# diaoenmao/Multimodal-Controller-for-Generative-Models

Hardware: AMD Instinct MI355X
Metric: images/sec (train step) MCGAN CIFAR-10 32x32 (higher is better)
Workload: dtype bf16

## Files before the change

### include/mcgen_hip.h

```cpp
#ifndef MCGEN_HIP_H
#define MCGEN_HIP_H

#include <stdint.h>

#ifdef __cplusplus
extern "C" {
#endif

enum { MCGEN_F32 = 0, MCGEN_BF16 = 1 };

const char* mcgen_last_error(void);
int mcgen_abi_version(void);

typedef struct {
    const void*  x;
    const float* scale;
    const float* shift;
    const float* code;
    const int16_t* cmap;
    int32_t C;
    int32_t ups;
    int32_t relu;
    int32_t ksize;
    int32_t group_n;
    int32_t cmap_stride;
    int32_t Cw;
    int32_t reserved_;
} mcgen_seg_t;

typedef struct {
    mcgen_seg_t  seg[2];
    int32_t      nseg;
    const void*  w;
    const float* bias;
    void*        y;
    int32_t N, H, W;
    int32_t Cout;
    int32_t Cout_w;
    int32_t Cy;
    int32_t pool;
    float   alpha;
    const void*  res;
    const float* ocode;
    const void*  gate_x;
    const float* gscale; const float* gshift; const float* gmean; const float* grstd;
    int32_t tanh_out;
    float*  stats;
    int32_t stats_mode;
    int32_t w_layout;
    const int16_t* ycmap;
    int32_t ycmap_stride;
    int32_t y_group;
    const float* bias2;
    const int32_t* wsel;
    int64_t wsel_stride;
    const int32_t* order;
    const int16_t* yperm;
    int32_t yperm_stride, reserved_;
} mcgen_conv_t;

enum { MCGEN_ROUTE_TILED = 0,
       MCGEN_ROUTE_MC, MCGEN_ROUTE_GK, MCGEN_ROUTE_GK_PP,
       MCGEN_ROUTE_SKINNY, MCGEN_ROUTE_SMAP, MCGEN_ROUTE_PX1, MCGEN_ROUTE_C8, MCGEN_ROUTE_HEAD };
typedef struct {
    int32_t route;
    int32_t form;
    int32_t bm, bn, pipe;
    int32_t m_tiles;
    int32_t grid_x, grid_y, threads, lds_bytes, a_bytes, grouped;
} mcgen_conv_plan_t;
int mcgen_conv_plan(const mcgen_conv_t* p, int dtype, mcgen_conv_plan_t* out);
int mcgen_conv_m_tiles(const mcgen_conv_t* p, int dtype);
int mcgen_conv_tile(const mcgen_conv_t* p, int dtype, int* bm, int* bn);
int mcgen_conv_form(const mcgen_conv_t* p, int dtype);
int mcgen_conv_fused(const mcgen_conv_t* p, int dtype, void* stream);

typedef struct {
    mcgen_seg_t  seg;
    const void*  dy;
    int32_t N, H, W;
    int32_t Cout, Cout_w, Cdy;
    int32_t dy_ups;
    float*  slabs;
    int32_t splits;
    int32_t halves;
    float*  bias_slabs;
} mcgen_wgrad_t;

int64_t mcgen_wgrad_slab_elems(const mcgen_wgrad_t* p);
int mcgen_wgrad(const mcgen_wgrad_t* p, int dtype, void* stream);
int mcgen_wgrad_c8_ok(const mcgen_wgrad_t* p, int dtype);
// ... 347 lines not shown
```

### multimodal-controller-for-generative-models_amd/csrc/conv_fused.hip

```cpp
#include "conv_tile.h"
#include <stdlib.h>
#include <type_traits>

namespace {

template <typename T, int BM, int BN, int WM, int WN>
struct ConvCfg {
    static constexpr int NT = 64 * WM * WN;
    static constexpr int FM = BM / WM / 16;
    static constexpr int FN = BN / WN / 16;
    static constexpr int ESZ = Elem<T>::BYTES;
    static constexpr int APITCH = MCGEN_CK * ESZ + 16 * ESZ;
    static constexpr int BROW = MCGEN_CK * ESZ;
    static constexpr int BBYTES = BN * BROW;
    static constexpr int EP = BN + 4;
    static constexpr int NI = (BM * 9 + NT - 1) / NT;
    static constexpr int UPR = BROW / 16;
    static constexpr int UNITS = BN * UPR;
    static constexpr int NU = (UNITS + NT - 1) / NT;
    static constexpr int EPX = (BN >= 128 && BM > 64) ? BM / 64 : 1;
    static constexpr int PPX = BM / EPX;
    static constexpr int CH = BN / 8;
    static constexpr int PROWS = NT / CH;
    static_assert(NT % CH == 0, "epilogue thread mapping");
// ... 1613 lines not shown
    int wset = 0;
    if (p.order || p.wsel) {
        const int tpi = (H * W) / BM, pos = tile_m / tpi;
        if (p.wsel) wset = p.wsel[pos];
        if (p.order) tile_m = p.order[pos] * tpi + (tile_m - pos * tpi);
    }
    const int cout0 = blockIdx.y * BN;
    const Geo g = make_geo(BM, tile_m, H, W);
    const int n_img = g.n0 < N ? g.n0 : N - 1;

    f32x4 acc[FN][FM];
#pragma unroll
    for (int i = 0; i < FN; ++i)
#pragma unroll
        for (int j = 0; j < FM; ++j) acc[i][j] = f32x4{0.f, 0.f, 0.f, 0.f};

    const mcgen_seg_t sg0 = seg_for_tile(p.seg[0], g);
    const int C0 = sg0.C;
    const char* wimg = reinterpret_cast<const char*>(p.w) + (size_t)wset * (size_t)p.wsel_stride * 2;
    const size_t wblock_bytes = (size_t)p.Cout_w * BROW;
    auto seg_info = [&](int si, const int16_t*& cidx, int& cw, int& cnt) {
        const mcgen_seg_t& sg = p.seg[si];
        cw = sg.Cw > 0 ? sg.Cw : sg.C;
        cidx = nullptr; cnt = sg.C;
        if (sg.cmap) {
            const int16_t* rec = sg.cmap + (size_t)n_img * sg.cmap_stride;
            cidx = rec + cw;
            cnt = (int)mc_sload(rec + 2 * cw + 32 + 2 * ((cw + 31) >> 5));
            if (cnt > sg.C) cnt = sg.C;
        }
    };
    const int16_t* cidx0 = nullptr; int cw0 = C0, cnt0 = C0;
    if constexpr (GK) seg_info(0, cidx0, cw0, cnt0);
    const int nchunk = GK ? ((cnt0 + 31) >> 5) : (C0 >> 5), T0 = nchunk * 9;
    const size_t tapstride0 = (size_t)(cw0 + 1) * p.Cout_w * 2;

    constexpr int UPR = C::UPR, RPP = 64 / UPR;
    int d_src[PPW];
    int k0_[PPW];
    const int rsub = lane / LPR, ci = lane % LPR;
#pragma unroll
    for (int k = 0; k < PPW; ++k) {
        const int piece = wave * PPW + k;
        if constexpr (!GK) {
            const int row = piece * RPP + lane / UPR, pu = lane % UPR;
            const int lgrp = pu ^ (3 * ((row >> 3) & 1));
            d_src[k] = (cout0 + row < p.Cout_w) ? (cout0 + row) * BROW + lgrp * 16 : (lane % UPR) * 16;
            k0_[k] = 0;
        } else {
            const int rho0 = RPPK * piece, rho = rho0 + rsub;
            k0_[k] = (rho0 < 16) ? 8 * (rho0 >> 2) + (rho0 & 3) : 8 * ((rho0 - 16) >> 2) + 4 + ((rho0 - 16) & 3);
            int co = cout0 + 16 * ((ci >> 1) ^ (rho & 7)) + 8 * (ci & 1);
            if (co > p.Cout_w - 8) co = p.Cout_w - 8;
            d_src[k] = co * 2;
        }
    }
    auto ksel_map = [&](const int16_t* cidx, int t, int k) -> int {
        const uint32_t d01 = mc_sload(cidx + 32 * t + k0_[k]);
        uint32_t sel = d01;
        if constexpr (RPPK == 4) {
            const uint32_t d23 = mc_sload(cidx + 32 * t + k0_[k] + 2);
            sel = (rsub & 2) ? d23 : d01;
        }
        return (int)((rsub & 1) ? (sel >> 16) : (sel & 0xffffu));
    };
    auto ksel = [&](const int16_t* cidx, int cw, int t, int k) -> int {
        if (cidx) return ksel_map(cidx, t, k);
// ... 164 lines not shown
                    for (int i = 0; i < HF; ++i) M::run(wf[fn], af[cs][i], acc[fn][i]);
            } else {
                const int sn = (slot_c + 1 == R) ? 0 : slot_c + 1;
                const char* ldsB = ldsB0 + sn * BB;
#pragma unroll
                for (int fn = 0; fn < FN; ++fn) {
#pragma unroll
                    for (int i = 0; i < HF; ++i) M::run(wf[fn], af[cs][i], acc[fn][HF + i]);
                    wf[fn] = wfrag(ldsB, fn);
                }
            }
            if constexpr (h == 0) {
                asm volatile("s_waitcnt lgkmcnt(0)" ::: "memory");
                pp_wait_vm<pp_vmcnt_b(ph, R, NIW, PPW)>();
                pp_barrier();
            } else {
                slot_c = (slot_c + 1 == R) ? 0 : slot_c + 1;
                ++tcur;
            }
        });
        if constexpr (GK) {
#pragma unroll
            for (int kk = 0; kk < PPW; ++kk) krow_c[kk] = krow_n[kk];
        }
    }
    asm volatile("s_waitcnt vmcnt(0)" ::: "memory");
    }

    if (p.nseg > 1) {
        int tg = 0;
        int nrest = 0;
        const int16_t* cidx1 = nullptr; int cw1 = 8, cnt1 = 0;
        if constexpr (GK) { seg_info(1, cidx1, cw1, cnt1); nrest = (cnt1 + 31) >> 5; }
        else for (int s = 1; s < p.nseg; ++s) nrest += (p.seg[s].C + MCGEN_CK - 1) / MCGEN_CK;
        const char* wseg1 = wimg + 9 * tapstride0;
        const size_t tapstride1 = (size_t)(cw1 + 1) * p.Cout_w * 2;
        auto tail_dma = [&](int t, int slot) {
#pragma unroll
            for (int k = 0; k < PPW; ++k) {
                if constexpr (GK) dma_piece_gk(wseg1, tapstride1, ksel(cidx1, cw1, t, k) * p.Cout_w * 2 + d_src[k], 0, slot, k);
                else dma_piece(T0 + t, slot, k);
            }
        };
        pp_barrier();
        constexpr int SUBW = BM * APITCH;
        constexpr int A2 = 2 * (((PP * APITCH + 1023) / 1024) * 1024);
        constexpr int TGMAX = (A2 + 2 * BB) / SUBW;
#ifndef MCGEN_PP_TG
#define MCGEN_PP_TG 4
#endif
        constexpr int TG = TGMAX < MCGEN_PP_TG ? TGMAX : MCGEN_PP_TG;
        constexpr int NI1 = (BM * 4 + NT - 1) / NT;
        static_assert(TG >= 1 && R >= 5, "tail groups: windows over the window buffers + two ring slots, weights in slots 2 .. 4");
        auto tslot = [](int t) { return 2 + t % 3; };
        auto tail_dma_c = [&](int t) { tail_dma(t < nrest ? t : nrest - 1, tslot(t)); };
        if (nrest > 0) { tail_dma_c(0); tail_dma_c(1); }
        for (int s = 1; s < p.nseg; ++s) {
            const mcgen_seg_t sg = seg_for_tile(p.seg[s], g);
            PatchStager<T, NT, NI1, APITCH> stager;
            stager.setup(sg, g, N, H, W, tid);
            const int b_lane = (wm * (BM / WM) + l15) * APITCH + lg * 16;
            const int nch = GK ? nrest : (sg.C + MCGEN_CK - 1) / MCGEN_CK;
#pragma unroll 1
            for (int q0 = 0; q0 < nch; q0 += TG) {
                const int ng = (nch - q0) < TG ? (nch - q0) : TG;
                if (q0 > 0) __builtin_amdgcn_s_barrier();
                {
                    typename PatchStager<T, NT, NI1, APITCH>::raw_t raw[TG];
#pragma unroll
                    for (int i = 0; i < TG; ++i) if (i < ng) stager.load(sg, (q0 + i) * MCGEN_CK, raw[i]);
#pragma unroll
                    for (int i = 0; i < TG; ++i) if (i < ng) stager.write(sg, (q0 + i) * MCGEN_CK, raw[i], ldsA0 + i * SUBW, g.n0 < N ? g.n0 : -1);
                }
#pragma unroll 1
                for (int i = 0; i < ng; ++i) {
                    if constexpr (PPW == 2) asm volatile("s_waitcnt vmcnt(2)" ::: "memory"); else asm volatile("s_waitcnt vmcnt(1)" ::: "memory");
                    asm volatile("s_waitcnt lgkmcnt(0)" ::: "memory");
                    pp_barrier();
                    tail_dma_c(tg + 2);
                    const char* ldsB = ldsB0 + tslot(tg) * BB;
                    const char* ldsW = ldsA0 + i * SUBW + b_lane;
                    typename M::frag xf[FM], yf[FN];
#pragma unroll
                    for (int fm = 0; fm < FM; ++fm) xf[fm] = *reinterpret_cast<const typename M::frag*>(ldsW + fm * 16 * APITCH);
#pragma unroll
                    for (int fn = 0; fn < FN; ++fn) yf[fn] = wfrag(ldsB, fn);
#pragma unroll
                    for (int fn = 0; fn < FN; ++fn)
#pragma unroll
                        for (int fm = 0; fm < FM; ++fm) M::run(yf[fn], xf[fm], acc[fn][fm]);
                    ++tg;
                }
            }
        }
    }
// ... 293 lines not shown
        r.route = MCGEN_ROUTE_C8;
    } else if (mcgen_conv_head_ok(p, dtype)) {
        r.route = MCGEN_ROUTE_HEAD;
    }
    const long Mtot = (long)p->N * p->H * p->W;
    r.m_tiles = r.route == MCGEN_ROUTE_SMAP ? p->N : bm > 0 ? (int)((Mtot + bm - 1) / bm) : 0;
    return r;
}
static int route_form(const Route& r) { return r.route >= MCGEN_ROUTE_SKINNY ? r.route - MCGEN_ROUTE_SKINNY + 1 : 0; }

static int validate(const mcgen_conv_t* p, bool launching) {
    MCGEN_CHECK(p && p->nseg >= 1 && p->nseg <= 2, "conv_fused: nseg must be 1 or 2");
    MCGEN_CHECK(p->N > 0 && ilog2_exact(p->H) >= 0 && ilog2_exact(p->W) >= 0, "conv_fused: H and W must be powers of two (got %dx%d)", p->H, p->W);
    MCGEN_CHECK(p->W <= 64 && p->H * p->W >= 1, "conv_fused: W up to 64 supported");
    MCGEN_CHECK(p->Cout > 0 && p->Cout_w == round_up(p->Cout, 16), "conv_fused: Cout_w must be Cout rounded up to 16");
    MCGEN_CHECK(p->Cy % 8 == 0 && p->Cy > 0, "conv_fused: Cy must be a positive multiple of 8");
    MCGEN_CHECK(p->w && p->y, "conv_fused: null weight image or output");
    for (int s = 0; s < p->nseg; ++s) {
        const mcgen_seg_t& g = p->seg[s];
        MCGEN_CHECK(g.x && g.C > 0 && g.C % 8 == 0, "conv_fused: segment %d: C must be a positive multiple of 8", s);
        MCGEN_CHECK(g.ksize == 1 || g.ksize == 3, "conv_fused: segment %d: ksize must be 1 or 3", s);
        MCGEN_CHECK(!g.ups || (p->H >= 2 && p->W >= 2), "conv_fused: upsampled segment needs H, W >= 2");
        MCGEN_CHECK(g.group_n >= 0 && (g.group_n == 0 || p->N % g.group_n == 0), "conv_fused: segment %d: group_n must divide N", s);
    }
    if (p->pool) MCGEN_CHECK(p->H >= 2 && p->W >= 2, "conv_fused: pooling needs H, W >= 2");
    MCGEN_CHECK(p->stats_mode >= 0 && p->stats_mode <= 2, "conv_fused: bad stats_mode");
    MCGEN_CHECK(p->stats_mode != 2 || (p->gate_x && p->gmean && p->grstd), "conv_fused: stats_mode 2 needs gate_x, gmean, grstd");
    MCGEN_CHECK(!launching || p->stats_mode == 0 || p->stats, "conv_fused: stats_mode set without a stats buffer");
    MCGEN_CHECK(p->w_layout >= 0 && p->w_layout <= 2, "conv_fused: unknown weight layout %d", p->w_layout);
    if (p->wsel || p->order) {
        MCGEN_CHECK(p->w_layout == 0 && (p->y_group == 0 || !p->order), "conv_fused: per-mode weight sets (wsel / order) go with the chunked weight image (w_layout 0)");
        MCGEN_CHECK(!p->wsel || p->wsel_stride > 0, "conv_fused: wsel needs wsel_stride");
    }
    if (p->yperm) {
        MCGEN_CHECK(p->wsel && !p->order && !p->ycmap, "conv_fused: permuted weight rows (yperm) come with wsel, without order / ycmap");
        MCGEN_CHECK(!p->pool && !p->res && !p->gate_x && !p->ocode && !p->tanh_out, "conv_fused: a compacted output takes bias and statistics only");
        MCGEN_CHECK(p->Cy % 8 == 0 && p->Cy <= p->Cout && p->Cout % 8 == 0 && p->Cout_w == p->Cout && p->Cout_w <= 256 && p->yperm_stride >= p->Cout && p->yperm_stride % 8 == 0,
                    "conv_fused: yperm: bad pitch %d / stride %d for %d channels", p->Cy, p->yperm_stride, p->Cout);
    }
    if (p->ycmap) {
        MCGEN_CHECK(!p->pool && !p->res && !p->gate_x && !p->ocode && !p->tanh_out && !p->bias2, "conv_fused: a compacted output takes bias and statistics only");
        MCGEN_CHECK(p->Cy % 32 == 0 && p->Cy <= round_up(p->Cout, 8) + 32 && p->ycmap_stride >= 2 * round_up(p->Cout, 8) + 32,
                    "conv_fused: compacted output: bad pitch %d / map stride %d", p->Cy, p->ycmap_stride);
        MCGEN_CHECK(p->Cout_w <= 256, "conv_fused: a compacted output needs all channels in one tile");
    } else if (!p->yperm) {
        MCGEN_CHECK(p->Cy >= p->Cout, "conv_fused: Cy must be >= Cout");
    }
    return 0;
}

static int check_mc(const mcgen_conv_t* p, int dtype, const TilePick& t) {
    MCGEN_CHECK(dtype == MCGEN_BF16, "conv_fused: K-major (mode-compacted) launches are bf16");
    for (int s = 0; s < p->nseg; ++s) {
        MCGEN_CHECK(p->seg[s].cmap && p->seg[s].cmap_stride >= 2 * p->seg[s].C + 32, "conv_fused: K-major launch: segment %d has no compaction map", s);
        MCGEN_CHECK(p->seg[s].C <= 2048, "conv_fused(mc): at most 2048 channels per segment");
    }
    MCGEN_CHECK(p->Cout_w % 8 == 0 && p->Cout_w >= 64, "conv_fused(mc): at least 64 output channels");
    MCGEN_CHECK(t.BM > 0, "conv_fused(mc): no tile of a %dx%d map lies inside one image", p->H, p->W);
    return 0;
}

static int check_gk(const mcgen_conv_t* p, int dtype, const TilePick& t) {
    MCGEN_CHECK(dtype == MCGEN_BF16, "conv_fused: K-major launches are bf16");
    for (int s = 0; s < p->nseg; ++s) {
        const mcgen_seg_t& g = p->seg[s];
        const int cw = g.Cw > 0 ? g.Cw : g.C;
// ... 108 lines not shown
```

### multimodal-controller-for-generative-models_amd/csrc/conv_head.hip

```cpp
#include "conv_tile.h"

namespace {

constexpr int HD_NT = 512, HD_W = 32, HD_ROWS = 8;
constexpr int HD_PC = HD_W + 2, HD_PP = (HD_ROWS + 2) * HD_PC;
constexpr int HD_PITCH = 80;
constexpr int HD_BUF = ((HD_PP * HD_PITCH + 127) / 128) * 128;
constexpr int HD_NI = (HD_PP * 4 + HD_NT - 1) / HD_NT;

__global__ __launch_bounds__(HD_NT, 4)
void conv_head_kernel(const mcgen_conv_t p) {
    extern __shared__ __attribute__((aligned(16))) char smem[];
    const int tid = threadIdx.x, lane = tid & 63;
    const int wv = __builtin_amdgcn_readfirstlane(tid >> 6);
    const int l15 = lane & 15, lg = lane >> 4;
    const int n = blockIdx.x >> 2, h0 = (blockIdx.x & 3) * HD_ROWS;
    const mcgen_seg_t sg = p.seg[0];
    const int C = sg.C, nchunk = C >> 5;
    const float* anyf = reinterpret_cast<const float*>(p.w);
    const size_t arow = sg.group_n > 0 ? (size_t)(n / sg.group_n) * C : 0;
    const float* scp = sg.scale ? sg.scale + arow : anyf;
    const float* shp = sg.scale ? sg.shift + arow : anyf;
    const float* cdp = sg.code ? sg.code + (size_t)n * C : anyf;
    const float relu_lo = sg.relu ? 0.f : -__builtin_inff();

    const int u = tid & 3;
    int src[HD_NI], dst[HD_NI];
#pragma unroll
    for (int k = 0; k < HD_NI; ++k) {
        const int wp = (tid >> 2) + 128 * k;
        const int wr = wp / HD_PC, wc = wp - wr * HD_PC;
        const int h = h0 + wr - 1, w = wc - 1;
        dst[k] = wp < HD_PP ? wp * HD_PITCH + u * 16 : -1;
        src[k] = (wp < HD_PP && (unsigned)h < (unsigned)HD_W && (unsigned)w < (unsigned)HD_W) ? ((n * HD_W + h) * HD_W + w) * C + u * 8 : -1;
    }
    const bf16_t* xs = reinterpret_cast<const bf16_t*>(sg.x);
    u32x4 raw[HD_NI];
    float sc[8], sh[8], cd[8];
    auto load_chunk = [&](int q) {
#pragma unroll
        for (int k = 0; k < HD_NI; ++k) raw[k] = *reinterpret_cast<const u32x4*>(xs + (src[k] >= 0 ? (size_t)src[k] + q * 32 : 0));
        load8f(sg.scale ? scp + q * 32 + u * 8 : anyf, sc);
        load8f(sg.scale ? shp + q * 32 + u * 8 : anyf, sh);
        load8f(sg.code ? cdp + q * 32 + u * 8 : anyf, cd);
    };
    auto write_chunk = [&](char* buf) {
#pragma unroll
        for (int k = 0; k < HD_NI; ++k) {
            if (dst[k] < 0) continue;
            union { bf16x8 h; u32x4 w; } o;
#pragma unroll
            for (int e = 0; e < 4; ++e) {
                const float s0 = sg.scale ? sc[2 * e] : 1.f, t0 = sg.scale ? sh[2 * e] : 0.f, c0 = sg.code ? cd[2 * e] : 1.f;
                const float s1 = sg.scale ? sc[2 * e + 1] : 1.f, t1 = sg.scale ? sh[2 * e + 1] : 0.f, c1 = sg.code ? cd[2 * e + 1] : 1.f;
                o.h[2 * e] = (bf16_t)(fmaxf(fmaf(__uint_as_float(raw[k][e] << 16), s0, t0), relu_lo) * c0);
                o.h[2 * e + 1] = (bf16_t)(fmaxf(fmaf(__uint_as_float(raw[k][e] & 0xffff0000u), s1, t1), relu_lo) * c1);
            }
            if (src[k] < 0) o.w = u32x4{0u, 0u, 0u, 0u};
            *reinterpret_cast<u32x4*>(buf + dst[k]) = o.w;
        }
    };

    f32x4 acc[2] = {f32x4{0.f, 0.f, 0.f, 0.f}, f32x4{0.f, 0.f, 0.f, 0.f}};
    const bf16_t* wimg = reinterpret_cast<const bf16_t*>(p.w) + (p.wsel ? (size_t)p.wsel[n] * (size_t)p.wsel_stride : 0) + (size_t)l15 * MCGEN_CK + lg * 8;
    load_chunk(0);
    write_chunk(smem);
#pragma unroll 1
    for (int q = 0; q < nchunk; ++q) {
        bf16x8 wf[9];
#pragma unroll
        for (int j = 0; j < 9; ++j) wf[j] = *reinterpret_cast<const bf16x8*>(wimg + ((size_t)(q * 9 + j) * 16) * MCGEN_CK);
        if (q + 1 < nchunk) load_chunk(q + 1);
        __syncthreads();
        const char* buf = smem + (q & 1) * HD_BUF;
#pragma unroll
        for (int j = 0; j < 9; ++j) {
#pragma unroll
            for (int f = 0; f < 2; ++f) {
                const bf16x8 xf = *reinterpret_cast<const bf16x8*>(buf + ((wv + j / 3) * HD_PC + 16 * f + l15 + j % 3) * HD_PITCH + lg * 16);
                acc[f] = __builtin_amdgcn_mfma_f32_16x16x32_bf16(wf[j], xf, acc[f], 0, 0, 0);
            }
        }
        if (q + 1 < nchunk) write_chunk(smem + ((q + 1) & 1) * HD_BUF);
    }
    if (lg < 2) {
        float bs[4];
#pragma unroll
        for (int r = 0; r < 4; ++r) {
            const int co = 4 * lg + r;
            bs[r] = (p.bias && co < p.Cout) ? p.bias[co] : 0.f;
            if (p.bias2 && co < p.Cout) bs[r] += p.bias2[co];
        }
        const int ny = p.y_group > 0 ? (n / p.y_group) * 2 * p.y_group + p.y_group + n % p.y_group : n;
        bf16_t* y = reinterpret_cast<bf16_t*>(p.y) + ((size_t)(ny * HD_W + h0 + wv) * HD_W) * p.Cy + 4 * lg;
#pragma unroll
        for (int f = 0; f < 2; ++f) {
            union { bf16_t h[4]; uint2 w; } o;
// ... 36 lines not shown
```

### multimodal-controller-for-generative-models_amd/csrc/small_ops.hip

```cpp
#include "mcgen_common.h"
#include <string.h>

static thread_local char g_err[512] = "";
int mcgen_fail(const char* fmt, ...) {
    va_list ap; va_start(ap, fmt); vsnprintf(g_err, sizeof(g_err), fmt, ap); va_end(ap);
    return 1;
}
extern "C" const char* mcgen_last_error(void) { return g_err; }
extern "C" int mcgen_abi_version(void) { return 9; }

namespace {

inline int grid_for(size_t n, int block = 256, int cap = 4096) {
    size_t b = (n + block - 1) / block; if (b < 1) b = 1; if (b > (size_t)cap) b = cap; return (int)b;
}
#define STREAM(s) reinterpret_cast<hipStream_t>(s)

template <typename T> __device__ __forceinline__ float ldf(const T* p) { return Elem<T>::to_f(*p); }

template <typename T>
__global__ void nchw_to_nhwc_kernel(const float* __restrict__ src, T* __restrict__ dst, int N, int C, int HW, int Cp) {
    const size_t total = (size_t)N * HW * Cp;
    for (size_t i = blockIdx.x * (size_t)blockDim.x + threadIdx.x; i < total; i += (size_t)gridDim.x * blockDim.x) {
        const int c = (int)(i % Cp); const size_t pix = i / Cp;
// ... 1117 lines not shown
                const unsigned k = i + e * bd;
                const float oa = (av[e] - da * ur[e] * vc[e]) * ia;
                const float ob = (bv[e] - db * ur2[e] * vc2[e]) * ib;
                float gi = oa + ob;
                if (wd != 0.f) gi = fmaf(wd, pv[e], gi);
                const float mi = fmaf(b1, mv[e], (1.f - b1) * gi);
                const float vi = fmaf(b2, vv[e], (1.f - b2) * gi * gi);
                M[k] = mi; V[k] = vi;
                P[k] = pv[e] - step_size * (mi / (sqrtf(vi) / bc2s + eps));
            }
        }
        for (; i < i1; i += bd) {
            const float oa = (A[i] - da * ua[r] * va[c]) * ia;
            const float ob = (B[i] - db * ub[r] * vb[c]) * ib;
            adam_elem(P, M, V, i, oa + ob, b1, b2, eps, wd, step_size, bc2s);
            c += dc; r += dr;
            if (c >= cols) { c -= cols; ++r; }
        }
    }
}

}

#define DISPATCH_T(dtype, CALL_F32, CALL_BF16) \
    if (dtype == MCGEN_F32) { CALL_F32; } else if (dtype == MCGEN_BF16) { CALL_BF16; } \
    else return mcgen_fail("unknown dtype %d", dtype)

namespace {
__global__ void onehot_rep_kernel(const int64_t* __restrict__ label, float* __restrict__ out, int* __restrict__ lab32, int n, int classes, int reps) {
    const int per = n * classes, total = per * reps;
    for (int i = blockIdx.x * blockDim.x + threadIdx.x; i < total; i += gridDim.x * blockDim.x) {
        const int e = i % per, row = e / classes, m = e - row * classes;
        out[i] = (label[row] == (int64_t)m) ? 1.f : 0.f;
        if (lab32 && m == 0) lab32[(i / per) * n + row] = (int)label[row];
    }
}
}
extern "C" int mcgen_onehot_rep(const int64_t* label, float* out, int* lab32, int N, int classes, int reps, void* stream) {
    MCGEN_CHECK(label && out && N > 0 && classes > 0 && reps > 0 && (long)N * classes * reps < (1L << 31), "onehot_rep: bad arguments");
    const int total = N * classes * reps;
    hipLaunchKernelGGL(onehot_rep_kernel, dim3(grid_for((size_t)total, 256, 256)), dim3(256), 0, STREAM(stream), label, out, lab32, N, classes, reps);
    MCGEN_LAUNCH_CHECK("onehot_rep"); return 0;
}
extern "C" int mcgen_nchw_to_nhwc(const float* src, void* dst, int dtype, int N, int C, int H, int W, int Cp, void* stream) {
    MCGEN_CHECK(src && dst && Cp >= C && Cp % 8 == 0, "nchw_to_nhwc: bad arguments");
    const size_t total = (size_t)N * H * W * Cp;
    DISPATCH_T(dtype,
        hipLaunchKernelGGL(nchw_to_nhwc_kernel<float>, dim3(grid_for(total)), dim3(256), 0, STREAM(stream), src, (float*)dst, N, C, H * W, Cp),
        hipLaunchKernelGGL(nchw_to_nhwc_kernel<bf16_t>, dim3(grid_for(total)), dim3(256), 0, STREAM(stream), src, (bf16_t*)dst, N, C, H * W, Cp));
    MCGEN_LAUNCH_CHECK("nchw_to_nhwc"); return 0;
}
extern "C" int mcgen_nhwc_to_nchw(const void* src, float* dst, int dtype, int N, int C, int H, int W, int Cp, void* stream) {
    MCGEN_CHECK(src && dst && Cp >= C, "nhwc_to_nchw: bad arguments");
    const size_t total = (size_t)N * H * W * C;
    DISPATCH_T(dtype,
        hipLaunchKernelGGL(nhwc_to_nchw_kernel<float>, dim3(grid_for(total)), dim3(256), 0, STREAM(stream), (const float*)src, dst, N, C, H * W, Cp),
        hipLaunchKernelGGL(nhwc_to_nchw_kernel<bf16_t>, dim3(grid_for(total)), dim3(256), 0, STREAM(stream), (const bf16_t*)src, dst, N, C, H * W, Cp));
    MCGEN_LAUNCH_CHECK("nhwc_to_nchw"); return 0;
}

extern "C" int mcgen_pool2_sum(const void* x, void* y, int dtype, int N, int Ho, int Wo, int C, void* stream) {
    MCGEN_CHECK(x && y && N > 0 && Ho > 0 && Wo > 0 && C > 0 && C % 8 == 0, "pool2_sum: bad arguments (C a multiple of 8)");
    const size_t total = (size_t)N * Ho * Wo * (C / 8);
    DISPATCH_T(dtype,
        hipLaunchKernelGGL(pool2_sum_kernel<float>, dim3(grid_for(total)), dim3(256), 0, STREAM(stream), (const float*)x, (float*)y, N, Ho, Wo, C),
        hipLaunchKernelGGL(pool2_sum_kernel<bf16_t>, dim3(grid_for(total)), dim3(256), 0, STREAM(stream), (const bf16_t*)x, (bf16_t*)y, N, Ho, Wo, C));
    MCGEN_LAUNCH_CHECK("pool2_sum"); return 0;
// ... 455 lines not shown
```

### multimodal-controller-for-generative-models_amd/gan_engine.py

```python
from __future__ import annotations

from typing import Dict, List, Optional

import torch
import torch.nn as nn

from . import gen_plan, ops
from ._lib import McgenError
from ._tuning import flag as _flag
from .ops import PrepJob, Seg

Tensor = torch.Tensor


def _bump(t: Tensor):
    torch.autograd.graph.increment_version(t)


class FlatState:

    def __init__(self, tensors: List[Tensor]):
        self.tensors = tensors
        self.flat: Optional[Tensor] = None
        self.offsets: List[int] = []
# ... 17 lines not shown
            flat = torch.zeros(total, dtype=torch.float32, device=dev)
            for t, off in zip(ts, offs):
                flat[off:off + t.numel()].copy_(t.detach().reshape(-1))
                t.data = flat[off:off + t.numel()].view(t.shape)
            self.flat, self.offsets = flat, offs
        return self.flat

    def offset_of(self, t: Tensor) -> int:
        return self.offsets[self._index[id(t)]]

    def view_of(self, flat: Tensor, t: Tensor) -> Tensor:
        off = self.offset_of(t)
        return flat[off:off + t.numel()].view(t.shape)

    def views(self, flat: Tensor) -> List[Tensor]:
        return [self.view_of(flat, t) for t in self.tensors]


class _BN:
    __slots__ = ('scale', 'shift', 'mean', 'rstd', 'count')


_PAIR_WGRAD = _flag('MCGEN_PAIR_WGRAD', '1') != '0'
_SN_FUSED = _flag('MCGEN_SN_FUSED', '0') == '1'
_SN_ROUNDS = _flag('MCGEN_SN_ROUNDS', '1') != '0'
_BUCKETS = _flag('MCGEN_BUCKETS', '1') != '0'
_MC = _flag('MCGEN_MC', '0') == '1'
_GK = _flag('MCGEN_GK', '1') != '0'
_LOWRES_SC_BWD = _flag('MCGEN_LOWRES_SC_BWD', '1') != '0'
_PM = _flag('MCGEN_PM', '1') != '0'
_PREP_CODES = _flag('MCGEN_PREP_CODES', '1') != '0'
_PM_HEAD = _flag('MCGEN_PM_HEAD', '1') != '0'
_PM_MAX_MODES = 16
class Nhwc:
    __slots__ = ('t', 'c')

    def __init__(self, t: Tensor, c: int):
        self.t, self.c = t, c

    @property
    def shape(self):
        n, h, w, _ = self.t.shape
        return torch.Size((n, self.c, h, w))


_SN_SNAP = _flag('MCGEN_SN_SNAP', '1') != '0'
_D0_FUSE = _flag('MCGEN_D0_FUSE', '1') != '0'
_BN_PAR = _flag('MCGEN_BN_PAR', '1') != '0'
_pending_counters: Dict[int, List[Tensor]] = {}
_pending_running: List = []


def _flush_counters():
    for k, ts in _pending_counters.items():
        if ts:
            torch._foreach_add_(ts, k)
    _pending_counters.clear()
    if _pending_running:
        ops.bn_running_batch(_pending_running)
        _pending_running.clear()


def _bn_forward(bn: nn.BatchNorm2d, stats: Optional[Tensor], count: int, train: bool, fold: int = 1, groups: int = 1) -> _BN:
    s = _BN()
    s.count = count
    if train:
# ... 118 lines not shown
            self._stack_plan = plan
        return self._stack

    def _gather_cmaps(self, plan, wsel):
        st, need = self._stacked_maps(plan), plan.pm_controllers
        if st is None:
            return {}
        idx = (wsel.view(1, -1) + st[1]).view(-1)
        rows = st[0].index_select(0, idx).view(len(need), wsel.numel(), st[0].shape[1])
        return {j: rows[k] for k, j in enumerate(need)}

    def _per_codebook(self, slot, mc, make):
        cb = mc.codebook
        key = (cb.data_ptr(), tuple(cb.shape), cb._version)
        cache = self.__dict__.setdefault('_cb_cache', {})
        if cache.get((slot, id(mc)), (None,))[0] != key:
            cache[slot, id(mc)] = (key, make(cb))
        return cache[slot, id(mc)][1]

    def _mode_perms(self, mc):
        return self._per_codebook('perms', mc, lambda cb: torch.argsort((cb == 0).to(torch.int8), dim=1, stable=True).to(torch.int16).contiguous())

    def _mode_maps(self, mc):
        return self._per_codebook('maps', mc, lambda cb: ops.mc_cmap(cb.detach().contiguous()))

    def _cap(self, mc):
        cb = mc.codebook
        if cb.is_cuda and torch.cuda.is_current_stream_capturing():
            raise McgenError('compacted generator pass: a codebook changed since the last eager pass; call '
                             'GeneratorEngine.warm_caps() before capturing (the compacted pitch is read on the host)')
        cap = (int((cb != 0).sum(1).max()) + 31) // 32 * 32
        return cap if cap <= cb.shape[1] * 3 // 4 and float(cb.min()) >= 0.0 else None

    def warm_caps(self):
        plan, mcs = self._plan(), self._codes.mcs
        for j in {j.kmap[0] for j in plan.jobs if j.kmap}:
            self._mode_maps(mcs[j])
        for j in {j.rmap[0] for j in plan.jobs if j.rmap}:
            self._mode_perms(mcs[j])
        self._stacked_maps(plan)

    def groups_supported(self, n_total: int, groups: int) -> bool:
        if groups <= 1:
            return True
        if n_total % groups:
            return False
        gn = n_total // groups
        lin, res, head_bn, head_mc, head_conv = self._layers()
        shapes = [(1, lin.out_features)]
        side = 4
        for b in res:
            side *= 2
            shapes += [(side, b.conv[4].module.out_channels)] * 2
        shapes.append((side, head_conv.out_channels))
        return all(gn % ops.tile_images(n_total, sd, sd, co, self.dtype) == 0 for sd, co in shapes)

    def forward(self, z: Tensor, indicator: Tensor, train: bool, groups: int = 1, nhwc: bool = False, one_hot: bool = False,
                pair_out: Optional[Tensor] = None):
        _pending_counters.clear(); _pending_running.clear()
        self.flat_p.ensure()
        lin, res, head_bn, head_mc, head_conv = self._layers()
        dt = self.dtype
        n = z.shape[0]
        if groups > 1 and not (train and self.groups_supported(n, groups)):
            raise RuntimeError(f'generator forward: {groups} statistics groups over {n} images is not supported')
        gn = n // groups if groups > 1 else 0
        ng = n // groups
        self.refresh_images()
        st_mode = 1 if train else 0
        ctx = {'train': train, 'n': n, 'groups': groups}
        zt = ops.to_nhwc(z.detach().reshape(n, -1, 1, 1), dt)
        c0 = lin.out_features // 16
        x0, st = ops.conv_fused([Seg(zt, ksize=1)], self.img['lin'], 16 * c0, bias=self.img['lin_bias'],
                                stats_mode=st_mode)
        x = x0.view(n, 4, 4, c0)
        fold = 16
        ctx['zt'] = zt
        blocks_ctx = []
        codes = self._codes.run_any(indicator)
        plan = self._plan()
        hint = getattr(indicator, '_mcgen_onehot', None)
        kind = 'plain'
        if groups > 1 and one_hot:
            kind = 'pm' if plan.pm_enabled and hint is not None and hint[0].shape[0] * hint[1] == n else 'gk'
        route = getattr(plan, kind)
        wsel, cmaps = None, {}
        if kind == 'pm':
            wsel = hint[2] if len(hint) > 2 and hint[2] is not None else hint[0].to(torch.int32).repeat(hint[1])
            cmaps = self._gather_cmaps(plan, wsel)

        def compacted(j, cap):
            return ((cmaps[j] if j in cmaps else ops.mc_cmap(codes[j])), cap) if cap else None

        def seg(x, code, cm, bn=None, gather=False, cmap=None, **kw):
            if cm is None:
                return Seg(x, scale=bn and bn.scale, shift=bn and bn.shift, code=code, group_n=gn if bn else 0, cmap=cmap, **kw)
            sc, sh = ops.mc_affine(code, cm[0], cm[1], bn and bn.scale, bn and bn.shift, group_n=gn if bn else 0)
            return Seg(x, scale=sc, shift=sh, group_n=1, **(dict(cmap=cm[0], cw=code.shape[1]) if gather else {}), **kw)

        x_cm = None
        for i, (b, r) in enumerate(zip(res, route.blocks)):
            s = x.shape[1]
            code1, code2 = codes[2 * i], codes[2 * i + 1]
            bn1 = _bn_forward(b.conv[0].module, st, ng * s * s, train, fold, groups)
            fold = 1
            conv_a, conv_b, conv_s = b.conv[4].module, b.conv[8].module, b.shortcut[2].module
            co = conv_a.out_channels
            cm_h = compacted(2 * i + 1, r.cap_h)
            cm_y = compacted(r.y_ctrl, r.cap_y)
            seg_a = seg(x, code1, x_cm, bn1, r.a.form == 'gk', ops.mc_cmap(code1) if r.a.form == 'mc' else None, ups=True, relu=True)
            how = dict(wsel=wsel, yperm=self._mode_perms(b.mc_2)) if r.a.form == 'pm' else \
                dict(kmajor=gen_plan.LAYOUT[r.a.form], ycmap=cm_h[0] if cm_h else None)
            h, st_h = ops.conv_fused([seg_a], self.img[r.a.image], co, bias=conv_a.bias, stats_mode=st_mode, cy=r.cap_h, **how)
            bn2 = _bn_forward(b.conv[5].module, st_h, ng * 4 * s * s, train, 1, groups)
            gk = r.b.form == 'gk'
            segs = [seg(h, code2, cm_h, bn2, gk, relu=True), seg(x, code1, x_cm, None, gk, ksize=1, ups=True)]
            if gk:
                how = dict(bias=conv_b.bias.detach() + conv_s.bias.detach(), kmajor=2, ycmap=cm_y[0] if cm_y else None)
            else:
                how = dict(bias=conv_b.bias, bias2=conv_s.bias)
                if r.b.form == 'pm':
                    how.update(wsel=wsel, yperm=self._mode_perms(self._codes.mcs[r.y_ctrl]) if cm_y else None)
            y, st = ops.conv_fused(segs, self.img[r.b.image], co, stats_mode=st_mode, cy=r.cap_y, **how)
            blocks_ctx.append(dict(x=x, h=h, code1=code1, code2=code2, bn1=bn1, bn2=bn2))
            x, x_cm = y, cm_y
        s = x.shape[1]
        bnh = _bn_forward(head_bn, st, ng * s * s, train, fold, groups)
        codeh = codes[-1]
        seg_h = seg(x, codeh, x_cm, bnh, relu=True)
        hw, hsel = self.img[route.head], (wsel if x_cm else None)
        cimg = head_conv.out_channels
        if pair_out is not None:
            if tuple(pair_out.shape) != (2 * n, x.shape[1], x.shape[2], ops.pad8(cimg)) or pair_out.dtype != dt:
                raise McgenError(f'pair_out must be {(2 * n, x.shape[1], x.shape[2], ops.pad8(cimg))} {dt}')
            direct = (dt == torch.bfloat16 and x.shape[1] == 32 and x.shape[2] == 32 and cimg <= 8 and x.shape[-1] % 32 == 0
                      and x.shape[-1] >= 64 and n * 32 * 32 * x.shape[-1] < (1 << 31))
            if direct:
                ops.conv_fused([seg_h], hw, cimg, bias=head_conv.bias, tanh=True, out=pair_out, y_group=ng, wsel=hsel)
                out = None
            else:
                out, _ = ops.conv_fused([seg_h], hw, cimg, bias=head_conv.bias, tanh=True, wsel=hsel)
                pv = pair_out.view(groups, 2 * ng, *pair_out.shape[1:])
                pv[:, ng:].copy_(out.view(groups, ng, *out.shape[1:]))
        else:
            out, _ = ops.conv_fused([seg_h], hw, cimg, bias=head_conv.bias, tanh=True, wsel=hsel)
        ctx.update(blocks=blocks_ctx, y=x, bnh=bnh, codeh=codeh, out=out)
        _flush_counters()
        if pair_out is not None:
            return None, ctx
        return (Nhwc(out, head_conv.out_channels) if nhwc else ops.to_nchw(out, head_conv.out_channels)), ctx

    def backward(self, ctx, dimg: Tensor, gflat: Tensor, accumulate: bool = False):
        for _ in self.backward_iter(ctx, dimg, gflat, accumulate, split=False):
            pass

    def bucket_cut(self) -> int:
        lin, res, head_bn, head_mc, head_conv = self._layers()
        return max(1, len(res) // 2) if len(res) > 1 else 0

    def backward_iter(self, ctx, dimg: Tensor, gflat: Tensor, accumulate: bool = False, split: bool = True):
        if not ctx['train']:
            raise RuntimeError('generator backward needs a training-mode forward (batch statistics)')
        if ctx.get('groups', 1) != 1:
            raise RuntimeError('a grouped generator pass is forward-only (its images feed discriminator updates detached)')
        lin, res, head_bn, head_mc, head_conv = self._layers()
        dt = self.dtype
        n = ctx['n']
        acc = accumulate
        out = ctx['out']
        self._prep_backward_images()
        dout = dimg.t if isinstance(dimg, Nhwc) else ops.to_nhwc(dimg.contiguous(), dt, out.shape[-1])
        dtn = ops.tanh_bwd(dout, out)
        y, bnh, codeh = ctx['y'], ctx['bnh'], ctx['codeh']
        c_img, c = head_conv.out_channels, head_conv.in_channels
        cut = self.bucket_cut()
        off_cut = self.flat_p.offset_of(next(p for p in res[cut].parameters())) if res else 0
        G = lambda p: self.flat_p.view_of(gflat, p)
        red = ops.deferred_reduces()
# ... 488 lines not shown
```

### multimodal-controller-for-generative-models_amd/ops.py

```python
from __future__ import annotations

import ctypes as C
import os as _os
from dataclasses import dataclass
from typing import NamedTuple, Optional, Sequence, Tuple

import torch

from . import _lib
from ._lib import check
from ._tuning import flag as _flag

Tensor = torch.Tensor


def _dt(dtype: torch.dtype) -> int:
    if dtype == torch.float32:
        return _lib.F32
    if dtype == torch.bfloat16:
        return _lib.BF16
    raise _lib.McgenError(f'unsupported compute dtype {dtype}')


def _stream() -> int:
# ... 254 lines not shown
    if out is None:
        out = torch.empty(n, dtype=dtype, device=w.device)
    assert out.numel() == n and out.dtype == dtype
    check(_lib.load().mcgen_prep_weight_k(_f32(w.contiguous()), _p(out), _dt(dtype), cout, cin, ks, _f32(sigma), float(wscale), _stream()),
          'prep_weight_k')
    return out


def weight_image_elems(cout: int, cin: int, ksize: int, transpose: bool = False) -> int:
    return int(_lib.load().mcgen_weight_image_elems(cout, cin, ksize, int(transpose)))


def prep_weight(w: Tensor, dtype: torch.dtype, transpose: bool = False, row_perm: int = 1,
                sigma: Optional[Tensor] = None, wscale: float = 1.0, out: Optional[Tensor] = None) -> Tensor:
    cout, cin = w.shape[0], w.shape[1]
    ks = w.shape[2] if w.dim() == 4 else 1
    n = weight_image_elems(cout, cin, ks, transpose)
    if out is None:
        out = torch.empty(n, dtype=dtype, device=w.device)
    assert out.numel() == n and out.dtype == dtype
    check(_lib.load().mcgen_prep_weight(_f32(w), _p(out), _dt(dtype), cout, cin, ks, int(transpose), row_perm,
                                        _f32(sigma), float(wscale), _stream()), 'prep_weight')
    return out


def conv_fused(segs: Sequence[Seg], wimg: Tensor, cout: int, *, bias: Optional[Tensor] = None, bias2: Optional[Tensor] = None,
               pool: bool = False, alpha: float = 1.0, res: Optional[Tensor] = None,
               ocode: Optional[Tensor] = None, gate_x: Optional[Tensor] = None,
               gscale: Optional[Tensor] = None, gshift: Optional[Tensor] = None,
               gmean: Optional[Tensor] = None, grstd: Optional[Tensor] = None,
               tanh: bool = False, stats_mode: int = 0, cy: Optional[int] = None,
               out: Optional[Tensor] = None, kmajor: int = 0, ycmap: Optional[Tensor] = None,
               y_group: int = 0, wsel: Optional[Tensor] = None, order: Optional[Tensor] = None,
               yperm: Optional[Tensor] = None) -> Tuple[Tensor, Optional[Tensor]]:
    s0 = segs[0]
    n = s0.x.shape[0]
    h = s0.x.shape[1] * (2 if s0.ups else 1)
    w = s0.x.shape[2] * (2 if s0.ups else 1)
    dtype = s0.x.dtype
    cy = cy or pad8(cout)
    ho, wo = (h // 2, w // 2) if pool else (h, w)
    p = _lib.Conv()
    p.nseg = len(segs)
    for i, s in enumerate(segs):
        if s.x.dtype != dtype:
            raise _lib.McgenError('all segments must share the compute dtype')
        hs = s.x.shape[1] * (2 if s.ups else 1)
        if hs != h or s.x.shape[0] != n:
            raise _lib.McgenError('segments disagree on the convolution resolution')
        s.fill(p.seg[i])
    if wimg.dtype != dtype:
        raise _lib.McgenError(f'weight image dtype {wimg.dtype} != activation dtype {dtype}')
    if kmajor:
        need = sum(s.ksize * s.ksize * ((s.cw or s.x.shape[-1]) + 1) for s in segs) * pad16(cout)
    else:
        need = sum(((s.x.shape[-1] + 31) // 32) * s.ksize * s.ksize for s in segs) * pad16(cout) * 32
    if wsel is not None:
        if wsel.dtype != torch.int32 or wsel.numel() != n or (order is not None and (order.dtype != torch.int32 or order.numel() != n)):
            raise _lib.McgenError('wsel / order must be int32 [N]')
        if wimg.numel() % need:
            raise _lib.McgenError(f'weight sets: {wimg.numel()} elements are not a multiple of one image ({need})')
    elif order is not None:
        raise _lib.McgenError('order comes with wsel')
    elif wimg.numel() != need:
        raise _lib.McgenError(f'weight image has {wimg.numel()} elements, the segments need {need}')
    y = out if out is not None else torch.empty((n, ho, wo, cy), dtype=dtype, device=s0.x.device)
    if y_group:
        if out is None or tuple(y.shape) != (2 * n, ho, wo, cy) or y.dtype != dtype or not y.is_contiguous():
            raise _lib.McgenError(f'y_group: `out` must be a contiguous {(2 * n, ho, wo, cy)} {dtype} buffer')
    else:
        assert tuple(y.shape) == (n, ho, wo, cy) and y.dtype == dtype
    p.w, p.bias, p.y = _p(wimg), _f32(bias), _p(y)
    p.bias2 = _f32(bias2)
    p.N, p.H, p.W = n, h, w
    p.Cout, p.Cout_w, p.Cy = cout, pad16(cout), cy
    p.pool, p.alpha = int(pool), float(alpha)
    for name, t in (('res', res), ('gate_x', gate_x)):
        if t is not None and (tuple(t.shape) != (n, ho, wo, cy) or t.dtype != dtype):
            raise _lib.McgenError(f'{name} must be {(n, ho, wo, cy)} {dtype}, got {tuple(t.shape)} {t.dtype}')
    if ocode is not None and tuple(ocode.shape) != (n, cout):
        raise _lib.McgenError(f'ocode must be {(n, cout)}')
    p.res, p.ocode, p.gate_x = _p(res), _f32(ocode), _p(gate_x)
    p.gscale, p.gshift, p.gmean, p.grstd = _f32(gscale), _f32(gshift), _f32(gmean), _f32(grstd)
    p.tanh_out, p.stats_mode = int(tanh), stats_mode
    p.w_layout = int(kmajor)
    p.y_group = int(y_group)
    p.wsel, p.wsel_stride, p.order = _p(wsel), (need if wsel is not None else 0), _p(order)
    p.yperm, p.yperm_stride = None, 0
    if yperm is not None:
        if wsel is None or yperm.dtype != torch.int16 or yperm.dim() != 2 or yperm.shape[0] * need != wimg.numel() or not yperm.is_contiguous():
            raise _lib.McgenError('yperm must be a contiguous int16 [sets, stride] table that comes with wsel')
        p.yperm, p.yperm_stride = _p(yperm), yperm.shape[1]
    p.ycmap, p.ycmap_stride = None, 0
    if ycmap is not None:
        if ycmap.dtype != torch.int16 or tuple(ycmap.shape) != (n, cmap_stride(pad8(cout))):
            raise _lib.McgenError(f'ycmap must be int16 {(n, cmap_stride(pad8(cout)))}')
        p.ycmap, p.ycmap_stride = _p(ycmap), ycmap.shape[1]
    stats = None
    lib = _lib.load()
    plan = _conv_plan(p, dtype)
    if stats_mode:
        stats = torch.empty((plan.m_tiles, 2, pad16(cout) if (ycmap is not None or yperm is not None) else cy), dtype=torch.float32, device=y.device)
        p.stats = _p(stats)
    kflops = 2.0 * n * h * w * cout * sum(s.ksize * s.ksize * s.x.shape[-1] for s in segs)

    def _name():
        base = f'conv_fused<{"bf16" if dtype == torch.bfloat16 else "f32"},{plan.bm},{plan.bn}{(",mc", ",gk")[kmajor - 1] if kmajor else ""}>'
        if plan.form:
            base = ('conv_skinny<bf16>', 'conv_smap<bf16>', 'conv_px1<bf16>', 'conv_c8<bf16>', 'conv_head<bf16>')[plan.form - 1]
        if _PROF_SHAPES:
            base += f' N{n} {h}x{w} ' + '+'.join(f'{s.x.shape[-1]}k{s.ksize}' for s in segs) + f'->{cout}' + \
                ('g' if gate_x is not None else '') + ('p' if pool else '') + (f's{stats_mode}' if stats_mode else '')
        return base
    if TILE_LOG is not None:
        bm, bn = C.c_int(plan.bm), C.c_int(plan.bn)
        if plan.form:
            check(lib.mcgen_conv_tile(C.byref(p), _dt(dtype), C.byref(bm), C.byref(bn)), 'conv_tile')
        TILE_LOG.append((bm.value, bn.value))
    if FORM_LOG is not None:
        FORM_LOG.append(kmajor)
    if KERNEL_LOG is not None:
        KERNEL_LOG.append(int(plan.form))
    _timed(_name, kflops, lambda: check(lib.mcgen_conv_fused(C.byref(p), _dt(dtype), _stream()), 'conv_fused'),
           lambda: _nbytes(wimg, y, res, gate_x, *[s.x for s in segs]))
    return y, stats
# ... 1615 lines not shown
```

Baseline: 18350.

## Skip dead input-channel chunks per mode in per-mode weight convolutions

Adds a per-weight-set table of live 32-channel chunk counts, computed from the multimodal controller codebooks (nonzero channels per mode). The fused conv and head kernels read the table and cap their K-loop chunk count for each segment, so chunks whose weights are zero for that mode are not loaded or multiplied. This relies on the per-mode weight image being laid out with live channels first, and it adds a host-built table that is refreshed when the plan changes. It also clamps labels in the one-hot kernel to guard indexing.

```diff
diff --git a/include/mcgen_hip.h b/include/mcgen_hip.h
--- a/include/mcgen_hip.h
+++ b/include/mcgen_hip.h
@@ -31,6 +31,7 @@
 typedef struct {
     mcgen_seg_t  seg[2];
     int32_t      nseg;
+    int32_t      yperm_stride;
     const void*  w;
     const float* bias;
     void*        y;
@@ -56,7 +57,7 @@
     int64_t wsel_stride;
     const int32_t* order;
     const int16_t* yperm;
-    int32_t yperm_stride, reserved_;
+    const int32_t* wlive;
 } mcgen_conv_t;
 
 enum { MCGEN_ROUTE_TILED = 0,
diff --git a/multimodal-controller-for-generative-models_amd/csrc/conv_fused.hip b/multimodal-controller-for-generative-models_amd/csrc/conv_fused.hip
--- a/multimodal-controller-for-generative-models_amd/csrc/conv_fused.hip
+++ b/multimodal-controller-for-generative-models_amd/csrc/conv_fused.hip
@@ -1669,7 +1669,14 @@
     };
     const int16_t* cidx0 = nullptr; int cw0 = C0, cnt0 = C0;
     if constexpr (GK) seg_info(0, cidx0, cw0, cnt0);
-    const int nchunk = GK ? ((cnt0 + 31) >> 5) : (C0 >> 5), T0 = nchunk * 9;
+    int nlive0 = C0 >> 5;
+    if constexpr (!GK) {
+        if (p.wlive) {
+            const int v = __builtin_amdgcn_readfirstlane(p.wlive[wset * p.nseg]);
+            nlive0 = v < 0 ? 0 : (v < nlive0 ? v : nlive0);
+        }
+    }
+    const int nchunk = GK ? ((cnt0 + 31) >> 5) : nlive0, T0 = nchunk * 9;
     const size_t tapstride0 = (size_t)(cw0 + 1) * p.Cout_w * 2;
 
     constexpr int UPR = C::UPR, RPP = 64 / UPR;
@@ -1900,14 +1907,21 @@
         int nrest = 0;
         const int16_t* cidx1 = nullptr; int cw1 = 8, cnt1 = 0;
         if constexpr (GK) { seg_info(1, cidx1, cw1, cnt1); nrest = (cnt1 + 31) >> 5; }
-        else for (int s = 1; s < p.nseg; ++s) nrest += (p.seg[s].C + MCGEN_CK - 1) / MCGEN_CK;
+        else {
+            nrest = (p.seg[1].C + MCGEN_CK - 1) / MCGEN_CK;
+            if (p.wlive) {
+                const int v = __builtin_amdgcn_readfirstlane(p.wlive[wset * p.nseg + 1]);
+                nrest = v < 0 ? 0 : (v < nrest ? v : nrest);
+            }
+        }
+        const int Tseg1 = (C0 >> 5) * 9;
         const char* wseg1 = wimg + 9 * tapstride0;
         const size_t tapstride1 = (size_t)(cw1 + 1) * p.Cout_w * 2;
         auto tail_dma = [&](int t, int slot) {
 #pragma unroll
             for (int k = 0; k < PPW; ++k) {
                 if constexpr (GK) dma_piece_gk(wseg1, tapstride1, ksel(cidx1, cw1, t, k) * p.Cout_w * 2 + d_src[k], 0, slot, k);
-                else dma_piece(T0 + t, slot, k);
+                else dma_piece(Tseg1 + t, slot, k);
             }
         };
         pp_barrier();
@@ -1928,7 +1942,7 @@
             PatchStager<T, NT, NI1, APITCH> stager;
             stager.setup(sg, g, N, H, W, tid);
             const int b_lane = (wm * (BM / WM) + l15) * APITCH + lg * 16;
-            const int nch = GK ? nrest : (sg.C + MCGEN_CK - 1) / MCGEN_CK;
+            const int nch = nrest;
 #pragma unroll 1
             for (int q0 = 0; q0 < nch; q0 += TG) {
                 const int ng = (nch - q0) < TG ? (nch - q0) : TG;
@@ -2288,6 +2302,7 @@
         MCGEN_CHECK(p->w_layout == 0 && (p->y_group == 0 || !p->order), "conv_fused: per-mode weight sets (wsel / order) go with the chunked weight image (w_layout 0)");
         MCGEN_CHECK(!p->wsel || p->wsel_stride > 0, "conv_fused: wsel needs wsel_stride");
     }
+    MCGEN_CHECK(!p->wlive || p->wsel, "conv_fused: live chunk counts (wlive) are per weight set: they come with wsel");
     if (p->yperm) {
         MCGEN_CHECK(p->wsel && !p->order && !p->ycmap, "conv_fused: permuted weight rows (yperm) come with wsel, without order / ycmap");
         MCGEN_CHECK(!p->pool && !p->res && !p->gate_x && !p->ocode && !p->tanh_out, "conv_fused: a compacted output takes bias and statistics only");
diff --git a/multimodal-controller-for-generative-models_amd/csrc/conv_head.hip b/multimodal-controller-for-generative-models_amd/csrc/conv_head.hip
--- a/multimodal-controller-for-generative-models_amd/csrc/conv_head.hip
+++ b/multimodal-controller-for-generative-models_amd/csrc/conv_head.hip
@@ -16,7 +16,13 @@
     const int l15 = lane & 15, lg = lane >> 4;
     const int n = blockIdx.x >> 2, h0 = (blockIdx.x & 3) * HD_ROWS;
     const mcgen_seg_t sg = p.seg[0];
-    const int C = sg.C, nchunk = C >> 5;
+    const int C = sg.C;
+    const int wset = p.wsel ? p.wsel[n] : 0;
+    int nchunk = C >> 5;
+    if (p.wlive) {
+        const int v = __builtin_amdgcn_readfirstlane(p.wlive[wset]);
+        nchunk = v < 0 ? 0 : (v < nchunk ? v : nchunk);
+    }
     const float* anyf = reinterpret_cast<const float*>(p.w);
     const size_t arow = sg.group_n > 0 ? (size_t)(n / sg.group_n) * C : 0;
     const float* scp = sg.scale ? sg.scale + arow : anyf;
@@ -62,7 +68,7 @@
     };
 
     f32x4 acc[2] = {f32x4{0.f, 0.f, 0.f, 0.f}, f32x4{0.f, 0.f, 0.f, 0.f}};
-    const bf16_t* wimg = reinterpret_cast<const bf16_t*>(p.w) + (p.wsel ? (size_t)p.wsel[n] * (size_t)p.wsel_stride : 0) + (size_t)l15 * MCGEN_CK + lg * 8;
+    const bf16_t* wimg = reinterpret_cast<const bf16_t*>(p.w) + (size_t)wset * (size_t)p.wsel_stride + (size_t)l15 * MCGEN_CK + lg * 8;
     load_chunk(0);
     write_chunk(smem);
 #pragma unroll 1
diff --git a/multimodal-controller-for-generative-models_amd/csrc/small_ops.hip b/multimodal-controller-for-generative-models_amd/csrc/small_ops.hip
--- a/multimodal-controller-for-generative-models_amd/csrc/small_ops.hip
+++ b/multimodal-controller-for-generative-models_amd/csrc/small_ops.hip
@@ -1173,7 +1173,10 @@
     for (int i = blockIdx.x * blockDim.x + threadIdx.x; i < total; i += gridDim.x * blockDim.x) {
         const int e = i % per, row = e / classes, m = e - row * classes;
         out[i] = (label[row] == (int64_t)m) ? 1.f : 0.f;
-        if (lab32 && m == 0) lab32[(i / per) * n + row] = (int)label[row];
+        if (lab32 && m == 0) {
+            const int64_t l = label[row];
+            lab32[(i / per) * n + row] = l < 0 ? 0 : (l >= (int64_t)classes ? classes - 1 : (int)l);
+        }
     }
 }
 }
diff --git a/multimodal-controller-for-generative-models_amd/gan_engine.py b/multimodal-controller-for-generative-models_amd/gan_engine.py
--- a/multimodal-controller-for-generative-models_amd/gan_engine.py
+++ b/multimodal-controller-for-generative-models_amd/gan_engine.py
@@ -73,6 +73,8 @@
 _PREP_CODES = _flag('MCGEN_PREP_CODES', '1') != '0'
 _PM_HEAD = _flag('MCGEN_PM_HEAD', '1') != '0'
 _PM_MAX_MODES = 16
+_PM_LIVE = _flag('MCGEN_PM_LIVE', '1') != '0'
+LIVE_ALL = 1 << 20
 class Nhwc:
     __slots__ = ('t', 'c')
 
@@ -257,6 +259,39 @@
         cap = (int((cb != 0).sum(1).max()) + 31) // 32 * 32
         return cap if cap <= cb.shape[1] * 3 // 4 and float(cb.min()) >= 0.0 else None
 
+    def live_chunks(self) -> Dict[str, Tensor]:
+        plan = self._plan()
+        if self.__dict__.get('_live_plan') is not plan:
+            mcs = self._codes.mcs
+            cb0 = mcs[0].codebook
+            if cb0.is_cuda and torch.cuda.is_current_stream_capturing():
+                raise McgenError('compacted generator pass: a codebook changed since the last eager pass; call '
+                                 'GeneratorEngine.warm_caps() before capturing')
+            modes = cb0.shape[0]
+            by_image: Dict[str, list] = {}
+            for j in plan.jobs:
+                by_image.setdefault(j.buffer, []).append(j)
+            old, self._live = self.__dict__.get('_live', {}), {}
+            chunks = {}
+            for name, jobs in by_image.items():
+                if not any(j.kmap for j in jobs):
+                    continue
+                nseg = len(jobs) // modes
+                cols = []
+                for j in jobs[:nseg]:
+                    c = j.kmap[0] if j.kmap else None
+                    if c is not None and c not in chunks:
+                        chunks[c] = ((mcs[c].codebook != 0).sum(1).to(torch.int32) + 31) // 32
+                    cols.append(chunks[c] if c is not None else torch.full((modes,), LIVE_ALL, dtype=torch.int32, device=cb0.device))
+                t = torch.stack(cols, 1).contiguous()
+                keep = old.get(name)
+                if keep is not None and keep.shape == t.shape and keep.device == t.device:
+                    keep.copy_(t)
+                    t = keep
+                self._live[name] = t
+            self._live_plan = plan
+        return self._live
+
     def warm_caps(self):
         plan, mcs = self._plan(), self._codes.mcs
         for j in {j.kmap[0] for j in plan.jobs if j.kmap}:
@@ -264,6 +299,7 @@
         for j in {j.rmap[0] for j in plan.jobs if j.rmap}:
             self._mode_perms(mcs[j])
         self._stacked_maps(plan)
+        self.live_chunks()
 
     def groups_supported(self, n_total: int, groups: int) -> bool:
         if groups <= 1:
@@ -313,6 +349,7 @@
         if kind == 'pm':
             wsel = hint[2] if len(hint) > 2 and hint[2] is not None else hint[0].to(torch.int32).repeat(hint[1])
             cmaps = self._gather_cmaps(plan, wsel)
+        live = self.live_chunks() if kind == 'pm' and _PM_LIVE else {}
 
         def compacted(j, cap):
             return ((cmaps[j] if j in cmaps else ops.mc_cmap(codes[j])), cap) if cap else None
@@ -334,7 +371,7 @@
             cm_h = compacted(2 * i + 1, r.cap_h)
             cm_y = compacted(r.y_ctrl, r.cap_y)
             seg_a = seg(x, code1, x_cm, bn1, r.a.form == 'gk', ops.mc_cmap(code1) if r.a.form == 'mc' else None, ups=True, relu=True)
-            how = dict(wsel=wsel, yperm=self._mode_perms(b.mc_2)) if r.a.form == 'pm' else \
+            how = dict(wsel=wsel, yperm=self._mode_perms(b.mc_2), wlive=live.get(r.a.image)) if r.a.form == 'pm' else \
                 dict(kmajor=gen_plan.LAYOUT[r.a.form], ycmap=cm_h[0] if cm_h else None)
             h, st_h = ops.conv_fused([seg_a], self.img[r.a.image], co, bias=conv_a.bias, stats_mode=st_mode, cy=r.cap_h, **how)
             bn2 = _bn_forward(b.conv[5].module, st_h, ng * 4 * s * s, train, 1, groups)
@@ -345,7 +382,7 @@
             else:
                 how = dict(bias=conv_b.bias, bias2=conv_s.bias)
                 if r.b.form == 'pm':
-                    how.update(wsel=wsel, yperm=self._mode_perms(self._codes.mcs[r.y_ctrl]) if cm_y else None)
+                    how.update(wsel=wsel, yperm=self._mode_perms(self._codes.mcs[r.y_ctrl]) if cm_y else None, wlive=live.get(r.b.image))
             y, st = ops.conv_fused(segs, self.img[r.b.image], co, stats_mode=st_mode, cy=r.cap_y, **how)
             blocks_ctx.append(dict(x=x, h=h, code1=code1, code2=code2, bn1=bn1, bn2=bn2))
             x, x_cm = y, cm_y
@@ -354,6 +391,7 @@
         codeh = codes[-1]
         seg_h = seg(x, codeh, x_cm, bnh, relu=True)
         hw, hsel = self.img[route.head], (wsel if x_cm else None)
+        hlive = live.get(route.head) if hsel is not None else None
         cimg = head_conv.out_channels
         if pair_out is not None:
             if tuple(pair_out.shape) != (2 * n, x.shape[1], x.shape[2], ops.pad8(cimg)) or pair_out.dtype != dt:
@@ -361,14 +399,14 @@
             direct = (dt == torch.bfloat16 and x.shape[1] == 32 and x.shape[2] == 32 and cimg <= 8 and x.shape[-1] % 32 == 0
                       and x.shape[-1] >= 64 and n * 32 * 32 * x.shape[-1] < (1 << 31))
             if direct:
-                ops.conv_fused([seg_h], hw, cimg, bias=head_conv.bias, tanh=True, out=pair_out, y_group=ng, wsel=hsel)
+                ops.conv_fused([seg_h], hw, cimg, bias=head_conv.bias, tanh=True, out=pair_out, y_group=ng, wsel=hsel, wlive=hlive)
                 out = None
             else:
-                out, _ = ops.conv_fused([seg_h], hw, cimg, bias=head_conv.bias, tanh=True, wsel=hsel)
+                out, _ = ops.conv_fused([seg_h], hw, cimg, bias=head_conv.bias, tanh=True, wsel=hsel, wlive=hlive)
                 pv = pair_out.view(groups, 2 * ng, *pair_out.shape[1:])
                 pv[:, ng:].copy_(out.view(groups, ng, *out.shape[1:]))
         else:
-            out, _ = ops.conv_fused([seg_h], hw, cimg, bias=head_conv.bias, tanh=True, wsel=hsel)
+            out, _ = ops.conv_fused([seg_h], hw, cimg, bias=head_conv.bias, tanh=True, wsel=hsel, wlive=hlive)
         ctx.update(blocks=blocks_ctx, y=x, bnh=bnh, codeh=codeh, out=out)
         _flush_counters()
         if pair_out is not None:
diff --git a/multimodal-controller-for-generative-models_amd/ops.py b/multimodal-controller-for-generative-models_amd/ops.py
--- a/multimodal-controller-for-generative-models_amd/ops.py
+++ b/multimodal-controller-for-generative-models_amd/ops.py
@@ -310,7 +310,7 @@
                tanh: bool = False, stats_mode: int = 0, cy: Optional[int] = None,
                out: Optional[Tensor] = None, kmajor: int = 0, ycmap: Optional[Tensor] = None,
                y_group: int = 0, wsel: Optional[Tensor] = None, order: Optional[Tensor] = None,
-               yperm: Optional[Tensor] = None) -> Tuple[Tensor, Optional[Tensor]]:
+               yperm: Optional[Tensor] = None, wlive: Optional[Tensor] = None) -> Tuple[Tensor, Optional[Tensor]]:
     s0 = segs[0]
     n = s0.x.shape[0]
     h = s0.x.shape[1] * (2 if s0.ups else 1)
@@ -369,6 +369,12 @@
         if wsel is None or yperm.dtype != torch.int16 or yperm.dim() != 2 or yperm.shape[0] * need != wimg.numel() or not yperm.is_contiguous():
             raise _lib.McgenError('yperm must be a contiguous int16 [sets, stride] table that comes with wsel')
         p.yperm, p.yperm_stride = _p(yperm), yperm.shape[1]
+    p.wlive = None
+    if wlive is not None:
+        if wsel is None or wlive.dtype != torch.int32 or not wlive.is_contiguous() or \
+                tuple(wlive.shape) != (wimg.numel() // need, len(segs)) or wlive.device != wimg.device:
+            raise _lib.McgenError('wlive must be a contiguous int32 [sets, segments] table that comes with wsel')
+        p.wlive = _p(wlive)
     p.ycmap, p.ycmap_stride = None, 0
     if ycmap is not None:
         if ycmap.dtype != torch.int16 or tuple(ycmap.shape) != (n, cmap_stride(pad8(cout))):
```

Measured after the change: 18550 (median of 6 runs). 1.01x the previous value.
